# SinOncology/BreakID

Measured on AMD Instinct MI355X. Metric: M reads/s clustered+split-scanned, higher is better.
Workload: dtype int32/u8 (+f64 sd replay)

## Files before the change

breakid_amd/capi.py:

```python
from __future__ import annotations

import ctypes as C
import math
import os
import subprocess

import numpy as np

from . import abi

_HERE = os.path.dirname(os.path.abspath(__file__))
LIB_PATH = os.path.join(_HERE, "libbreakid_hip.so")
_LIB = None


class BreakIDError(RuntimeError):
    def __init__(self, code, msg):
        super().__init__("libbreakid_hip error %d: %s" % (code, msg))
        self.code = code


def build(verbose=False):
    cmd = ["make", "-C", os.path.join(_HERE, "csrc"), "-j8"]
    r = subprocess.run(cmd, capture_output=not verbose, text=True)
    if r.returncode != 0:
        raise RuntimeError("building libbreakid_hip.so failed:\n" + (r.stdout or "")[-4000:] + (r.stderr or "")[-4000:])


EXPORTS = ["bk_init", "bk_prepare_process", "bk_free", "bk_last_error", "bk_set_stream", "bk_sync", "bk_get_stream", "bk_upload_records", "bk_records", "bk_exclude_regions", "bk_isize_stats",
           "bk_discordant_pairs", "bk_mask_and_cluster", "bk_split_evidence", "bk_cluster_summary",
           "bk_split_breakpoints", "bk_normal_support", "bk_ref_support", "bk_genotype_call", "bk_clip_support", "bk_clip_reads", "bk_base_depth", "bk_clip_rescue", "bk_junctions", "bk_junction_sides", "bk_vcf_breakend_alt", "bk_evidence", "bk_unique_support", "bk_clip_consensus", "bk_junction_fit", "bk_locus_similarity", "bk_site_complexity", "bk_window_coverage", "bk_window_context", "bk_call_windows", "bk_fusion_frame", "bk_link_calls", "bk_locus_partners", "bk_call_partner_sites", "bk_fragment_sizes", "bk_fragment_bounds", "bk_known_calls", "bk_split_junctions", "bk_split_junction_counts", "bk_debug_split_junctions", "bk_cigar_gaps", "bk_cigar_gap_counts", "bk_clip_loci", "bk_clip_locus_counts", "bk_run", "bk_fetch", "bk_timing", "bk_timing_enable", "bk_timing_touched", "bk_group_stats", "bk_qname_hash", "bk_qname_check",
           "bk_bam_open", "bk_bam_header", "bk_bam_decode", "bk_bam_close", "bk_bam_extract", "bk_bam_names_free", "bk_bam_reads", "bk_reads_free", "bk_bam_decode_device", "bk_bam_decode_device_part", "bk_bam_decode_device_ctx", "bk_bam_dev_free", "bk_feed_release_caches", "bk_debug_bgzf_inflate", "bk_debug_std_sort", "bk_debug_scan", "bk_debug_radix_sort", "bk_debug_prims_info", "bk_sort_forms", "bk_debug_sort_info", "bk_debug_ahc", "bk_debug_points", "bk_debug_points_groups", "bk_debug_cluster_info", "bk_debug_stream_info", "bk_debug_stream_blocks", "bk_debug_cigar", "bk_debug_vote", "bk_debug_region", "bk_shard_begin", "bk_shard_get_stats", "bk_shard_set_stats",
           "bk_shard_sd_local", "bk_shard_sd_finish", "bk_shard_buffer", "bk_shard_set_buffer", "bk_shard_group_sizes",
           "bk_shard_own_groups", "bk_shard_route_candidates", "bk_shard_group_keys", "bk_shard_route_pairs", "bk_shard_group_pairs", "bk_shard_bp_cov", "bk_shard_bp_vote", "bk_shard_bp_vote_slice", "bk_shard_bp_set_voted", "bk_shard_bp_depth", "bk_shard_bp_finish"]


def lib():
    global _LIB
    if _LIB is None:
        if not os.path.exists(LIB_PATH):
            raise BreakIDError(abi.BK_ERR_NO_DEVICE, "libbreakid_hip.so is not built (run __graft_entry__.build()); "
                                                     "there is no CPU fallback")
        try:
            import torch
        except Exception:
            pass
        L = C.CDLL(LIB_PATH)
# ... 46 lines not shown
        L.bk_cigar_gaps.argtypes = [vp, C.c_int, C.c_uint32, C.c_uint32, C.c_uint32, C.c_uint32, C.POINTER(vp), u64p]
        L.bk_cigar_gap_counts.argtypes = [vp, u64p]
        L.bk_clip_loci.argtypes = [vp, vp, C.c_int, C.c_int, C.c_uint32, C.c_uint32, C.c_uint32, C.POINTER(vp), u64p]
        L.bk_clip_locus_counts.argtypes = [vp, u64p]
        L.bk_fetch.argtypes = [vp, C.c_int, C.POINTER(vp), u64p, C.POINTER(C.POINTER(C.c_uint64)), C.POINTER(C.c_uint32)]
        L.bk_timing.argtypes = [vp, C.POINTER(C.POINTER(C.c_char_p)), C.POINTER(C.POINTER(C.c_float)),
                                C.POINTER(C.POINTER(C.c_uint64)), C.POINTER(C.c_int)]
        L.bk_timing_enable.argtypes = [vp, C.c_int]
        L.bk_timing_touched.argtypes = [vp, C.POINTER(C.POINTER(C.c_uint64)), C.POINTER(C.c_int)]
        L.bk_debug_std_sort.argtypes = [vp, vp, vp, C.c_uint32, vp]
        L.bk_debug_scan.argtypes = [vp, C.c_int, vp, C.c_uint64, C.c_int, vp]
        L.bk_debug_radix_sort.argtypes = [vp, vp, vp, C.c_uint64, C.c_int, C.c_int, vp, vp]
        L.bk_debug_prims_info.argtypes = [u64p]
        L.bk_sort_forms.argtypes = [vp, u64p]
        L.bk_debug_sort_info.argtypes = [vp, u64p]
        L.bk_debug_ahc.argtypes = [vp, vp, vp, C.c_uint32, C.c_double, vp, vp, C.POINTER(C.c_uint32)]
        L.bk_debug_points.argtypes = [vp, C.c_int, vp, vp, C.c_uint32, C.c_double, vp, vp, C.POINTER(C.c_uint32)]
        L.bk_debug_points_groups.argtypes = [vp, C.c_int, vp, vp, vp, C.c_uint32, C.c_double, vp, vp, vp, C.POINTER(C.c_uint32)]
        L.bk_debug_cluster_info.argtypes = [u64p]
        L.bk_debug_stream_info.argtypes = [u64p]
        L.bk_debug_stream_blocks.argtypes = [C.c_uint]
        L.bk_debug_cigar.argtypes = [vp, C.c_uint32, vp, vp, vp, vp, vp, vp, vp]
        L.bk_debug_vote.argtypes = [vp, vp, C.c_uint32, vp, C.c_uint32, C.c_int32, C.c_int32, vp]
        L.bk_debug_region.argtypes = [vp, C.c_int32, C.c_uint32, C.c_uint32, C.c_uint64, vp, C.c_uint32, C.POINTER(C.c_uint32), C.POINTER(C.c_uint32),
                                      C.POINTER(C.c_uint32)]
        L.bk_shard_begin.argtypes = [vp, C.c_uint64, C.c_int]
        L.bk_shard_get_stats.argtypes = [vp, C.POINTER(abi.ShardStats)]
        L.bk_shard_set_stats.argtypes = [vp, C.POINTER(abi.ShardStats)]
        L.bk_shard_sd_local.argtypes = [vp, u64p, C.POINTER(vp), u64p]
        L.bk_shard_sd_finish.argtypes = [vp, vp, C.c_uint64, C.c_uint64, dp, dp]
# ... 108 lines not shown

def stream_info():
    out = (C.c_uint64 * 4)()
    rc = lib().bk_debug_stream_info(out)
    if rc != 0:
        raise BreakIDError(rc, "bk_debug_stream_info")
    return dict(zip(("STREAM_V", "ST_CAND_CAP", "ST_SA_CAP", "RESIDENT"), (int(v) for v in out)))


def stream_blocks(blocks):
    rc = lib().bk_debug_stream_blocks(int(blocks))
    if rc != 0:
        raise BreakIDError(rc, "bk_debug_stream_blocks")


def w_from(mean, sd):
    times = 2
    return times * math.sqrt(times) * (mean + 3 * sd)


def genotype_call(alt, ref):
    gt, gq, vaf = C.c_uint8(), C.c_uint8(), C.c_float()
    rc = lib().bk_genotype_call(int(alt), int(ref), C.byref(gt), C.byref(gq), C.byref(vaf))
    if rc != 0:
        raise BreakIDError(rc, "bk_genotype_call")
    return gt.value, gq.value, np.float32(vaf.value)


def junction_sides(row):
    a = np.zeros(1, abi.JUNCTION)
# ... 832 lines not shown
```

breakid_amd/csrc/api.hip:

```cpp
#include <algorithm>
#include <cmath>
#include <limits>
#include <cstring>
#include <numeric>

#include "bk_common.h"
#include "prims.h"
#include "stream.h"
#include "join.h"
#include "cluster.h"
#include "bp.h"
#include "normal.h"
#include "genotype.h"
#include "clip.h"
#include "junction.h"
#include "evidence.h"
#include "unique.h"
#include "consensus.h"
#include "jfit.h"
#include "locsim.h"
#include "seqcx.h"
#include "coverage.h"
#include "context.h"
#include "frame.h"
#include "link.h"
#include "partners.h"
#include "fragsize.h"
#include "known.h"
#include "sjcall.h"
#include "gaps.h"
#include "cliploci.h"
#include "exclude.h"
#include "ahc.h"
#include "lanes.h"
#include "bgzf_gpu.h"

namespace
{
thread_local std::string g_init_error;

uint64_t fnv64(const std::string &s)
{
  uint64_t h = 0xCBF29CE484222325ull;
  for (unsigned char c : s)
  {
    h ^= c;
    h *= 0x100000001B3ull;
  }
  return h;
// ... 27 lines not shown
  std::vector<int32_t> hdr_id_host;
  DevBuf d_tprefix, d_nhash, d_nid, d_own, d_hdr;
  NameTableDev names{};

  bk_soa rec{};
  DevBuf col[13];
  DevBuf d_side;
  DevBuf xcol[13];
  bool have_records = false;
  bool streamed = false;

  DevBuf d_counters, d_sd, d_cand, d_split_raw, d_split, d_sa_list;
  StreamCounters hc{};
  SdState hsd{};
  bool stream_done = false, splits_sorted = false;
  int mapq_min = 20;
  int stream_mapq = -1;
  uint64_t cand_cap = 0, split_cap = 0, sa_cap = 0;
  uint64_t rec_base = 0;
  std::vector<uint64_t> route_counts;
  JoinBufs jb2;
  const Cand *ext_cand = nullptr;
  const bk_split *ext_split = nullptr;
  bk_cluster *ext_clusters = nullptr;
  std::vector<uint8_t> own_groups;
  const Cand *cand_ptr() const { return ext_cand ? ext_cand : d_cand.get<Cand>(); }
  const bk_split *split_raw_ptr() const { return ext_split ? ext_split : d_split_raw.get<bk_split>(); }
  bk_cluster *clusters_ptr() const { return ext_clusters ? ext_clusters : d_clusters.get<bk_cluster>(); }
  SdBufs sdb;
  double mean = 0, sd = 0;
// ... 71 lines not shown
  ClipLociStats cll_stats;
  std::vector<struct bk_clip_locus> f_cll;

  prims::RadixBufs dbg_radix;
  DevBuf dbg_in, dbg_out, dbg_vals;

  std::vector<bk_pair> f_pairs[3];
  std::vector<uint64_t> f_off[3];
  std::vector<bk_split> f_splits;
  std::vector<bk_cluster> f_clusters;
  std::vector<int32_t> f_gkeys;
  std::vector<bk_group_stat> f_gstats;

  bool timing = false;
  std::vector<StageTimer> timers;
  Timing tout;

  void tick(const char *name, uint64_t bytes, bool begin, uint64_t touched = 0)
  {
    if (!timing) return;
    if (begin)
    {
      StageTimer t;
      t.name = name;
      t.bytes = bytes;
      t.touched = touched;
      HIP_CHECK(hipEventCreate(&t.a));
      HIP_CHECK(hipEventCreate(&t.b));
      HIP_CHECK(hipEventRecord(t.a, st));
      timers.push_back(t);
    }
    else
      HIP_CHECK(hipEventRecord(timers.back().b, st));
  }
};

static RecView rec_view(const bk_ctx *ctx)
{
  RecView r;
  r.n = ctx->rec.n;
  r.tid = ctx->rec.tid; r.pos = ctx->rec.pos; r.flag = ctx->rec.flag; r.mapq = ctx->rec.mapq;
  r.cigar_off = ctx->rec.cigar_off; r.cigar = ctx->rec.cigar;
  r.isize = ctx->rec.isize; r.aux_off = ctx->rec.aux_off;
  return r;
}

namespace
{
struct Scope
{
  bk_ctx *c;
  Scope(bk_ctx *c, const char *name, uint64_t bytes = 0, uint64_t touched = 0) : c(c) { c->tick(name, bytes, true, touched); }
  ~Scope()
  {
    try
    {
      c->tick("", 0, false);
    }
    catch (...)
    {
    }
  }
};

template <class F> int guarded(bk_ctx *ctx, F &&f)
{
  if (!ctx) return BK_ERR_ARG;
  try
  {
    HIP_CHECK(hipSetDevice(ctx->device));
    f();
    return BK_OK;
// ... 106 lines not shown
  (void) c->d_sa_list.as<uint32_t>(c->sa_cap);
}
bool stream_finish(bk_ctx *c)
{
  HIP_CHECK(hipMemcpyAsync(&c->hc, c->d_counters.get<StreamCounters>(), sizeof(StreamCounters), hipMemcpyDeviceToHost, c->st));
  HIP_CHECK(hipMemcpyAsync(&c->hsd, c->d_sd.get<SdState>(), sizeof(SdState), hipMemcpyDeviceToHost, c->st));
  HIP_CHECK(hipStreamSynchronize(c->st));
  if (c->hc.n_cand > c->cand_cap || c->hc.n_sa > c->sa_cap)
  {
    c->cand_cap = std::max<uint64_t>(c->cand_cap, c->hc.n_cand + 1024);
    c->sa_cap = std::max<uint64_t>(c->sa_cap, c->hc.n_sa + 1024);
    return false;
  }
  return true;
}
void stream_rare_path(bk_ctx *c)
{
  const uint64_t n = c->rec.n;
  if (c->timing && !c->timers.empty())
  {
    c->timers.back().bytes += 32ull * c->hc.n_cand + 4ull * c->hc.n_sa;
    c->timers.back().touched = 23ull * n + 4ull * c->rec.n_cigar_words + (c->rec.qcheck ? 60ull : 56ull) * c->hc.n_cand + 4ull * c->hc.n_sa;
  }
  if (c->hc.unsorted) throw bk_error(BK_ERR_UNSORTED, "records are not coordinate sorted (the reference requires an indexed, sorted BAM)");
  if (c->hc.n_sa > c->split_cap)
  {
    c->split_cap = c->hc.n_sa + 1024;
    (void) c->d_split_raw.as<bk_split>(c->split_cap);
  }
  StreamArgs a = stream_args(c, n);
  {
    Scope s(c, "k_split_records", c->rec.n_aux_bytes + 4ull * c->hc.n_sa);
    launch_split_records(a, c->hc.n_sa, c->st);
  }
  HIP_CHECK(hipMemcpyAsync(&c->hc, c->d_counters.get<StreamCounters>(), sizeof(StreamCounters), hipMemcpyDeviceToHost, c->st));
  HIP_CHECK(hipStreamSynchronize(c->st));
  if (c->timing && !c->timers.empty())
  {
    c->timers.back().bytes += 48ull * c->hc.n_split;
    c->timers.back().touched = c->timers.back().bytes + 40ull * c->hc.n_sa + 32ull * c->hc.n_split;
  }
  c->stream_done = true;
  c->stream_mapq = c->mapq_min;
  c->splits_sorted = false;
  c->stats_done = false;
}

void run_stream(bk_ctx *c)
{
  if (!c->have_records) throw bk_error(BK_ERR_ARG, "no records uploaded");
  const uint64_t n = c->rec.n;
  for (int attempt = 0; attempt < 3; ++attempt)
  {
    stream_prepare(c, n);
    {
      Scope s(c, "k_stream", 39ull * n + 4ull * c->rec.n_cigar_words);
      launch_stream(stream_args(c, n), c->st);
    }
    if (stream_finish(c)) break;
    if (c->timing && !c->timers.empty()) c->timers.pop_back();
    if (attempt == 2) throw bk_error(BK_ERR_LIMIT, "stream pass: output capacity");
  }
  stream_rare_path(c);
}

void ensure_splits_sorted(bk_ctx *c)
{
  if (c->splits_sorted) return;
  Scope s(c, "split_sort");
  bk_split *sorted = c->d_split.as<bk_split>(c->hc.n_split + 1);
  int bits = 0;
  if (!c->ext_split && c->rec_base == 0)
  {
    bits = 1;
    while (bits < 32 && (1ull << bits) < c->rec.n) ++bits;
  }
  sort_splits(const_cast<bk_split *>(c->split_raw_ptr()), c->hc.n_split, sorted, c->bb, c->st, bits);
  c->splits_sorted = true;
}
}

extern "C" {

void bk_prepare_process()
{
  static std::once_flag once;
  std::call_once(once, [] {
    const char *q = getenv("GPU_MAX_HW_QUEUES");
    stage_set_hw_queues(q ? atoi(q) : 4);
  });
}

// ... 310 lines not shown
        ctx->jb.rec_bits = bits;
      }
      join_candidates(ctx->cand_ptr(), ctx->hc.n_cand, w, ctx->d_tprefix.get<uint32_t>(), ctx->nt, ctx->jb, ctx->st, ctx->jr);
    }
    finish_groups(ctx, nullptr);
    ctx->clustered = false;
    ctx->joined = true;
    ctx->bp_done = false;
    ctx->sj_claims_valid = false;
    ctx->join_w = w;
    if (n_pairs) *n_pairs = ctx->jr.n_pairs;
    if (n_groups) *n_groups = ctx->jr.n_groups;
  });
}

int bk_mask_and_cluster(bk_ctx *ctx, double w, int fast, uint64_t *n_clustered)
{
  return guarded(ctx, [&] {
    const StageInput in{ctx->device, ctx->st, ctx->jr, ctx->gstart_host, ctx->own_groups,
                        [&](const char *name, const std::function<void()> &body) { Scope s(ctx, name); body(); }};
    ctx->summary_map = false;
    ctx->stage.run(in, w, fast);
    ctx->clustered = true;
    if (n_clustered) *n_clustered = ctx->stage.list.n;
  });
}

int bk_split_evidence(bk_ctx *ctx, uint64_t *n_tuples)
{
  return guarded(ctx, [&] {
    if (!ctx->stream_done) run_stream(ctx);
    ensure_splits_sorted(ctx);
    if (n_tuples) *n_tuples = ctx->hc.n_split;
  });
}

int bk_cluster_summary(bk_ctx *ctx, double w, uint64_t *n_clusters)
{
  return guarded(ctx, [&] {
    if (!ctx->clustered) throw bk_error(BK_ERR_ARG, "bk_cluster_summary: call bk_mask_and_cluster first");
    ctx->bp_done = false;
// ... 1271 lines not shown
{
  if (!mate_chr || !buf) return BK_ERR_ARG;
  const char br = mate_right ? '[' : ']';
  const std::string mate = br + std::string(mate_chr) + ":" + std::to_string(mate_pos) + br;
  const std::string alt = own_right ? mate + ref_base : ref_base + mate;
  if (alt.size() + 1 > cap) return BK_ERR_ARG;
  std::memcpy(buf, alt.c_str(), alt.size() + 1);
  return BK_OK;
}

int bk_run(bk_ctx *ctx, int mapq_min, int fast, double *w_out, uint64_t *n_valid)
{
  if (!ctx) return BK_ERR_ARG;
  if (ctx->stream_done && mapq_min != ctx->stream_mapq) ctx->stream_done = false;
  ctx->mapq_min = mapq_min;
  double mean, sd;
  int rc = bk_isize_stats(ctx, &mean, &sd);
  if (rc) return rc;
  const int times = 2;
  const double w = times * std::sqrt(times) * (mean + 3 * sd);
  if (w_out) *w_out = w;
  if ((rc = bk_discordant_pairs(ctx, mapq_min, w, nullptr, nullptr))) return rc;
  if ((rc = bk_mask_and_cluster(ctx, w, fast, nullptr))) return rc;
  if ((rc = bk_split_evidence(ctx, nullptr))) return rc;
  if ((rc = bk_cluster_summary(ctx, w, nullptr))) return rc;
  if ((rc = bk_split_breakpoints(ctx, w, n_valid))) return rc;
  return BK_OK;
}

int bk_fetch(bk_ctx *ctx, int stage, const void **data, uint64_t *count, const uint64_t **group_off, uint32_t *n_groups)
{
  return guarded(ctx, [&] {
    if (!data || !count) throw bk_error(BK_ERR_ARG, "bk_fetch: null output");
    const uint32_t ng = ctx->jr.n_groups;
    if (group_off) *group_off = nullptr;
    if (n_groups) *n_groups = 0;
    auto fetch_list = [&](int slot, const uint32_t *d_idx, const uint64_t *d_goff, const uint32_t *d_cl, uint64_t n) {
      std::vector<bk_pair> all(ctx->jr.n_pairs);
// ... 406 lines not shown
    if (!out) throw bk_error(BK_ERR_ARG, "bk_sort_forms: null output");
    ctx->stage.sort_forms(out);
  });
}

int bk_debug_sort_info(bk_ctx *ctx, uint64_t out[13])
{
  return guarded(ctx, [&] {
    if (!out) throw bk_error(BK_ERR_ARG, "bk_debug_sort_info: null output");
    static_assert(SORT_INFO_WORDS == 11, "bk_debug_sort_info: eleven words of the build, two of the last sort");
    std_sort_info(out);
    const SortEmuBufs &se = ctx->stage.cb().se;
    out[11] = se.last_heap[0];
    out[12] = se.last_heap[1];
  });
}

int bk_debug_ahc(bk_ctx *ctx, const uint32_t *x, const uint32_t *y, uint32_t n, double w, uint32_t *idx_out, int32_t *cluster_out, uint32_t *n_out)
{
  return guarded(ctx, [&] {
    if (!x || !y || !idx_out || !cluster_out || !n_out) throw bk_error(BK_ERR_ARG, "bk_debug_ahc: null argument");
    std::vector<bk_pair> hp(n);
    for (uint32_t i = 0; i < n; ++i)
    {
      memset(&hp[i], 0, sizeof(bk_pair));
      hp[i].x = x[i];
      hp[i].y = y[i];
    }
    DevBuf dp, dcl;
    PairList L;
// ... 435 lines not shown
```

breakid_amd/csrc/lanes.h:

```cpp
#pragma once
#include <functional>
#include <memory>

#include "join.h"
#include "cluster.h"
#include "ahc.h"

void stage_set_hw_queues(int n);

struct StageInput
{
  int device;
  hipStream_t st;
  const JoinResult &jr;
  const std::vector<uint64_t> &gstart_host;
  const std::vector<uint8_t> &own_groups;
  std::function<void(const char *name, const std::function<void()> &body)> timed;
};

struct ClusterStage
{
  SortService svc;
  std::vector<hipEvent_t> svc_probe;
  int svc_late = 0;
  bool svc_refused = false;
  struct Lane
  {
    ClusterBufs cb;
    PairList list, iso;
    DevBuf d_cluster;
    hipStream_t st = nullptr;
    ~Lane()
// ... 19 lines not shown
```

breakid_amd/csrc/lanes.hip:

```cpp
#include <algorithm>
#include <atomic>
#include <chrono>
#include <cmath>
#include <cstdio>
#include <numeric>
#include <thread>
#include <dirent.h>

#include "lanes.h"

static int g_hw_queues_at_init = 0;
void stage_set_hw_queues(int n) { g_hw_queues_at_init = n; }

static bool sort_service_on()
{
  static const bool on = !(getenv("BREAKID_SORT_SERVICE") && atoi(getenv("BREAKID_SORT_SERVICE")) == 0);
  return on;
}
constexpr int LANE_STREAMS_MAX = 4;
constexpr int SVC_STAGE_QUEUES = LANE_STREAMS_MAX + 3;
static bool lane_service(int fast) { return sort_service_on() && fast && g_hw_queues_at_init >= SVC_STAGE_QUEUES; }
static int stage_queues() { return std::max(1, g_hw_queues_at_init - 1); }
static int lanes_wanted(bool svc)
{
// ... 213 lines not shown
{
  uint32_t *ii = idx.as<uint32_t>(L.n + 1), *ig = gof ? gof->as<uint32_t>(L.n + 1) : nullptr;
  uint64_t *io = goff.as<uint64_t>((uint64_t) L.ng + 1);
  if (L.n) HIP_CHECK(hipMemcpyAsync(ii, L.idx.get<uint32_t>(), L.n * 4, hipMemcpyDeviceToDevice, st));
  if (L.n && ig) HIP_CHECK(hipMemcpyAsync(ig, L.gof.get<uint32_t>(), L.n * 4, hipMemcpyDeviceToDevice, st));
  if (L.ng) HIP_CHECK(hipMemcpyAsync(io, L.goff.get<uint64_t>(), ((uint64_t) L.ng + 1) * 8, hipMemcpyDeviceToDevice, st));
}
static void cluster_list(const bk_pair *pairs, PairList &L, double w, int fast, DevBuf &cl, ClusterBufs &cb, AhcBufs &ab, hipStream_t st)
{
  if (fast)
    fast_cluster_all(pairs, L, w, cl, cb, st);
  else
    ahc_cluster_all(pairs, L, w, cl, ab, cb, st);
}

using LanePlan = std::vector<int>;
static LanePlan plan_owned(const StageInput &in)
{
  const uint32_t ng = in.jr.n_groups;
  const bool owned_only = !in.own_groups.empty();
  if (owned_only && in.own_groups.size() != ng) throw bk_error(BK_ERR_ARG, "bk_shard_own_groups: group count changed");
  LanePlan p(ng, 0);
  for (uint32_t g = 0; owned_only && g < ng; ++g)
    if (!in.own_groups[g]) p[g] = -1;
  return p;
}
static LanePlan plan_blind(const StageInput &in, int K)
{
  const uint32_t ng = in.jr.n_groups;
  std::vector<uint32_t> order(ng);
  std::iota(order.begin(), order.end(), 0u);
  auto size_of = [&](uint32_t g) { return in.gstart_host[g + 1] - in.gstart_host[g]; };
  std::stable_sort(order.begin(), order.end(), [&](uint32_t a, uint32_t b) { return size_of(a) > size_of(b); });
  constexpr double wexp = 2.0;
  LanePlan p = plan_owned(in);
  std::vector<double> load(K, 0.0);
  for (uint32_t i = 0; i < ng; ++i)
  {
    const uint32_t g = order[i];
    if (p[g] < 0) continue;
    int l = 0;
    for (int k = 1; k < K; ++k)
      if (load[k] < load[l]) l = k;
    load[l] += std::pow((double) size_of(g), wexp);
    p[g] = l;
  }
  return p;
}
static LanePlan plan_observed(const std::vector<uint64_t> &sizes, const std::vector<uint32_t> &hx, const std::vector<uint32_t> &hy, int K)
{
  const uint32_t ng = (uint32_t) sizes.size();
  constexpr double per_pair = 0.001;
  auto heap_cost = [](uint32_t m) { return (double) m + (m > 40947u ? 1.0 * (double) (m - 40947u) : 0.0); };
  std::vector<uint32_t> order(ng);
  std::iota(order.begin(), order.end(), 0u);
  auto chain = [&](uint32_t g) { return heap_cost(hx[g]) + heap_cost(hy[g]); };
  std::stable_sort(order.begin(), order.end(), [&](uint32_t a, uint32_t b) {
    const double ca = chain(a), cb = chain(b);
    return ca != cb ? ca > cb : sizes[a] > sizes[b];
  });
  LanePlan p(ng, 0);
  std::vector<double> mx(K, 0.0), my(K, 0.0), pairs(K, 0.0);
  auto cost = [&](int l) { return mx[l] + my[l] + per_pair * pairs[l]; };
  for (uint32_t g : order)
  {
    int best = 0;
    double best_cost = 0;
    for (int l = 0; l < K; ++l)
    {
      const double c = std::max(mx[l], heap_cost(hx[g])) + std::max(my[l], heap_cost(hy[g])) + per_pair * (pairs[l] + (double) sizes[g]);
      if (l == 0 || c < best_cost || (c == best_cost && cost(l) < cost(best)))
      {
        best = l;
        best_cost = c;
      }
    }
    mx[best] = std::max(mx[best], heap_cost(hx[g]));
    my[best] = std::max(my[best], heap_cost(hy[g]));
    pairs[best] += (double) sizes[g];
    p[g] = best;
  }
  if (bk_debug("lanes"))
    for (int l = 0; l < K; ++l)
    {
      fprintf(stderr, "[lanes] lane %d: max heap x %.0f y %.0f, %.0f pairs, cost %.0f; heavy groups:", l, mx[l], my[l], pairs[l], cost(l));
      for (uint32_t g = 0; g < ng; ++g)
        if (p[g] == l && (hx[g] || hy[g])) fprintf(stderr, " %u(%u,%u)", g, hx[g], hy[g]);
      fprintf(stderr, "\n");
    }
  return p;
}
static uint32_t *upload_drop(const LanePlan &p, int K, DevBuf &buf, hipStream_t st)
{
  const size_t row = p.size() + 1;
  std::vector<uint32_t> drop((size_t) K * row, 0u);
  for (int l = 0; l < K; ++l)
    for (size_t g = 0; g + 1 < row; ++g) drop[(size_t) l * row + g] = p[g] == l ? 0u : 1u;
  uint32_t *d = buf.as<uint32_t>(drop.size() + 1);
  HIP_CHECK(hipMemcpyAsync(d, drop.data(), drop.size() * 4, hipMemcpyHostToDevice, st));
  HIP_CHECK(hipStreamSynchronize(st));
  return d;
}

static void group_lanes(ClusterStage &cs, const StageInput &in, double w, int fast)
// ... 97 lines not shown
    if (observe) cb.heavy_x.assign(ng, 0u);
    remove_isolated_end(pairs, lane(l).list, cb, lane_st(l));
    if (observe) cb.observe = false;
  };
  auto cluster_lane = [&](int l) {
    PairList &L = lane(l).list, &iso = lane(l).iso;
    iso.n = L.n;
    iso.ng = L.ng;
    snapshot_list(L, iso.idx, &iso.gof, iso.goff, lane_st(l));
    cluster_list(pairs, L, w, fast, lane(l).d_cluster, lane(l).cb, cs.ab, lane_st(l));
  };
  const auto tp0 = std::chrono::steady_clock::now();
  auto phase = [&](const char *what) {
    if (dbg) fprintf(stderr, "[lanes] %s at %.2f ms\n", what, std::chrono::duration<double, std::milli>(std::chrono::steady_clock::now() - tp0).count());
  };
  upload_plan(plan_blind(in, K));
  phase("plan uploaded");
  if (use_svc)
    in_lanes([&](int l) {
      mask_lane(l, false);
      cluster_lane(l);
    });
  else
  {
    in_lanes([&](int l) { mask_lane(l, true); });
    PairList &mid = cs.lane_mid;
    merge_all(&ClusterStage::Lane::list, mid, nullptr);
    std::vector<uint64_t> goff_h((size_t) ng + 1);
    HIP_CHECK(hipMemcpyAsync(goff_h.data(), mid.goff.get<uint64_t>(), ((size_t) ng + 1) * 8, hipMemcpyDeviceToHost, in.st));
    HIP_CHECK(hipStreamSynchronize(in.st));
    std::vector<uint64_t> sizes(ng);
    std::vector<uint32_t> hx(ng, 0u), hy(ng, 0u);
    for (uint32_t g = 0; g < ng; ++g) sizes[g] = goff_h[g + 1] - goff_h[g];
    for (int l = 0; l < K; ++l)
      for (uint32_t g = 0; g < ng; ++g)
      {
        hx[g] = std::max(hx[g], lane(l).cb.heavy_x[g]);
        hy[g] = std::max(hy[g], lane(l).cb.heavy_y[g]);
      }
    upload_plan(plan_observed(sizes, hx, hy, K));
    in_lanes([&](int l) {
      list_subset_ranges(mid, goff_h.data(), keep[l].data(), lane(l).list, lane_st(l));
      cluster_lane(l);
    });
  }
  phase("lanes done");
  svc_stage.finish();
  phase("service stopped");
  if (use_svc && bk_debug("lanes")) fprintf(stderr, "[svc] tasks: %u wide, %u narrow\n", cs.svc.stats[0], cs.svc.stats[1]);
  PairList &iso_m = cs.lane_iso_m;
  merge_all(&ClusterStage::Lane::iso, iso_m, nullptr);
  merge_all(&ClusterStage::Lane::list, cs.list, &cs.d_cluster);
  HIP_CHECK(hipStreamSynchronize(in.st));
  phase("lists merged");
  cs.iso_n = iso_m.n;
// ... 40 lines not shown
```

include/breakid_hip.h:

```cpp
#ifndef BREAKID_HIP_H
#define BREAKID_HIP_H

#include <stdint.h>
#include <stddef.h>

#ifdef __cplusplus
extern "C" {
#endif

#define BK_OK 0
#define BK_ERR_ARG (-1)
#define BK_ERR_HIP (-2)
#define BK_ERR_NO_DEVICE (-3)
#define BK_ERR_UNSORTED (-4)
#define BK_ERR_CIGAR (-5)
#define BK_ERR_IO (-6)
#define BK_ERR_LIMIT (-7)
#define BK_ERR_COLLISION (-8)

#define BK_MEM_HOST 0
#define BK_MEM_DEVICE 1

typedef struct bk_ctx bk_ctx;

// ... 350 lines not shown
int bk_shard_bp_vote_slice(bk_ctx *ctx, double w, const void *cov_total_dev, uint64_t lo, uint64_t hi, void **clusters_dev, void **voted_dev);
int bk_shard_bp_set_voted(bk_ctx *ctx, const void *voted_all_dev);
int bk_shard_bp_depth(bk_ctx *ctx, void **depth_dev, uint64_t *n);
int bk_shard_bp_finish(bk_ctx *ctx, const void *depth_total_dev);

int bk_debug_std_sort(bk_ctx *ctx, const uint32_t *key, const uint64_t *group_off, uint32_t n_groups, uint32_t *perm_out);

int bk_debug_scan(bk_ctx *ctx, int elem_bytes, const void *in, uint64_t n, int in_place, void *out);
int bk_debug_radix_sort(bk_ctx *ctx, const uint64_t *keys, const uint32_t *vals, uint64_t n, int begin_bit, int end_bit, uint64_t *keys_out, uint32_t *vals_out);
int bk_debug_prims_info(uint64_t out[4]);

int bk_sort_forms(bk_ctx *ctx, uint64_t out[3]);

int bk_debug_sort_info(bk_ctx *ctx, uint64_t out[13]);

int bk_debug_ahc(bk_ctx *ctx, const uint32_t *x, const uint32_t *y, uint32_t n, double w, uint32_t *idx_out, int32_t *cluster_out, uint32_t *n_out);

int bk_debug_points(bk_ctx *ctx, int mode, const uint32_t *x, const uint32_t *y, uint32_t n, double w, uint32_t *idx_out, int32_t *cluster_out, uint32_t *n_out);
int bk_debug_points_groups(bk_ctx *ctx, int mode, const uint32_t *x, const uint32_t *y, const uint64_t *group_off, uint32_t n_groups, double w, uint32_t *idx_out,
                           int32_t *cluster_out, uint64_t *goff_out, uint32_t *n_out);
int bk_debug_cluster_info(uint64_t out[2]);
int bk_debug_stream_info(uint64_t out[4]);
int bk_debug_stream_blocks(unsigned blocks);
int bk_debug_cigar(bk_ctx *ctx, uint32_t n, const uint8_t *kind, const uint32_t *c1_off, const uint8_t *c1, const uint32_t *c2_off, const uint8_t *c2, const int32_t *e,
                   int32_t *out6);
int bk_debug_vote(bk_ctx *ctx, const bk_split *side1, uint32_t n1, const bk_split *side2, uint32_t n2, int32_t p1_tid, int32_t p2_tid, int32_t *out3);
int bk_debug_region(bk_ctx *ctx, int32_t tid, uint32_t start, uint32_t end, uint64_t depth_pos, bk_split *out, uint32_t cap, uint32_t *n_out, uint32_t *cov_out,
                    uint32_t *depth_out);

typedef struct bk_bam bk_bam;
// ... 30 lines not shown
```

Baseline: 11730.

## Overlap split-record extraction with clustering lanes and model-based lane dealing

```diff
diff --git a/breakid_amd/capi.py b/breakid_amd/capi.py
--- a/breakid_amd/capi.py
+++ b/breakid_amd/capi.py
@@ -30,7 +30,7 @@
 EXPORTS = ["bk_init", "bk_prepare_process", "bk_free", "bk_last_error", "bk_set_stream", "bk_sync", "bk_get_stream", "bk_upload_records", "bk_records", "bk_exclude_regions", "bk_isize_stats",
            "bk_discordant_pairs", "bk_mask_and_cluster", "bk_split_evidence", "bk_cluster_summary",
            "bk_split_breakpoints", "bk_normal_support", "bk_ref_support", "bk_genotype_call", "bk_clip_support", "bk_clip_reads", "bk_base_depth", "bk_clip_rescue", "bk_junctions", "bk_junction_sides", "bk_vcf_breakend_alt", "bk_evidence", "bk_unique_support", "bk_clip_consensus", "bk_junction_fit", "bk_locus_similarity", "bk_site_complexity", "bk_window_coverage", "bk_window_context", "bk_call_windows", "bk_fusion_frame", "bk_link_calls", "bk_locus_partners", "bk_call_partner_sites", "bk_fragment_sizes", "bk_fragment_bounds", "bk_known_calls", "bk_split_junctions", "bk_split_junction_counts", "bk_debug_split_junctions", "bk_cigar_gaps", "bk_cigar_gap_counts", "bk_clip_loci", "bk_clip_locus_counts", "bk_run", "bk_fetch", "bk_timing", "bk_timing_enable", "bk_timing_touched", "bk_group_stats", "bk_qname_hash", "bk_qname_check",
-           "bk_bam_open", "bk_bam_header", "bk_bam_decode", "bk_bam_close", "bk_bam_extract", "bk_bam_names_free", "bk_bam_reads", "bk_reads_free", "bk_bam_decode_device", "bk_bam_decode_device_part", "bk_bam_decode_device_ctx", "bk_bam_dev_free", "bk_feed_release_caches", "bk_debug_bgzf_inflate", "bk_debug_std_sort", "bk_debug_scan", "bk_debug_radix_sort", "bk_debug_prims_info", "bk_sort_forms", "bk_debug_sort_info", "bk_debug_ahc", "bk_debug_points", "bk_debug_points_groups", "bk_debug_cluster_info", "bk_debug_stream_info", "bk_debug_stream_blocks", "bk_debug_cigar", "bk_debug_vote", "bk_debug_region", "bk_shard_begin", "bk_shard_get_stats", "bk_shard_set_stats",
+           "bk_bam_open", "bk_bam_header", "bk_bam_decode", "bk_bam_close", "bk_bam_extract", "bk_bam_names_free", "bk_bam_reads", "bk_reads_free", "bk_bam_decode_device", "bk_bam_decode_device_part", "bk_bam_decode_device_ctx", "bk_bam_dev_free", "bk_feed_release_caches", "bk_debug_bgzf_inflate", "bk_debug_std_sort", "bk_debug_scan", "bk_debug_radix_sort", "bk_debug_prims_info", "bk_sort_forms", "bk_debug_sort_info", "bk_debug_lane_plan", "bk_debug_ahc", "bk_debug_points", "bk_debug_points_groups", "bk_debug_cluster_info", "bk_debug_stream_info", "bk_debug_stream_blocks", "bk_debug_cigar", "bk_debug_vote", "bk_debug_region", "bk_shard_begin", "bk_shard_get_stats", "bk_shard_set_stats",
            "bk_shard_sd_local", "bk_shard_sd_finish", "bk_shard_buffer", "bk_shard_set_buffer", "bk_shard_group_sizes",
            "bk_shard_own_groups", "bk_shard_route_candidates", "bk_shard_group_keys", "bk_shard_route_pairs", "bk_shard_group_pairs", "bk_shard_bp_cov", "bk_shard_bp_vote", "bk_shard_bp_vote_slice", "bk_shard_bp_set_voted", "bk_shard_bp_depth", "bk_shard_bp_finish"]
 
@@ -107,6 +107,7 @@
         L.bk_debug_prims_info.argtypes = [u64p]
         L.bk_sort_forms.argtypes = [vp, u64p]
         L.bk_debug_sort_info.argtypes = [vp, u64p]
+        L.bk_debug_lane_plan.argtypes = [vp, vp, vp, C.c_uint32, C.c_int, C.c_int, vp, vp]
         L.bk_debug_ahc.argtypes = [vp, vp, vp, C.c_uint32, C.c_double, vp, vp, C.POINTER(C.c_uint32)]
         L.bk_debug_points.argtypes = [vp, C.c_int, vp, vp, C.c_uint32, C.c_double, vp, vp, C.POINTER(C.c_uint32)]
         L.bk_debug_points_groups.argtypes = [vp, C.c_int, vp, vp, vp, C.c_uint32, C.c_double, vp, vp, vp, C.POINTER(C.c_uint32)]
@@ -245,6 +246,23 @@
         raise BreakIDError(rc, "bk_debug_stream_blocks")
 
 
+LANE_PLAN_GREEDY, LANE_PLAN_MODEL, LANE_PLAN_EVAL = 0, 1, 2
+
+
+def lane_plan(pairs, hx, hy, K, which=LANE_PLAN_MODEL, plan=None):
+    pairs = np.ascontiguousarray(pairs, np.uint64)
+    hx = np.ascontiguousarray(hx, np.uint32)
+    hy = np.ascontiguousarray(hy, np.uint32)
+    assert len(pairs) == len(hx) == len(hy)
+    lane = np.zeros(len(pairs), np.int32) if plan is None else np.array(plan, np.int32)
+    assert len(lane) == len(pairs) and (which == LANE_PLAN_EVAL) == (plan is not None)
+    t = np.zeros(K, np.float64)
+    rc = lib().bk_debug_lane_plan(pairs.ctypes.data, hx.ctypes.data, hy.ctypes.data, len(pairs), int(K), int(which), lane.ctypes.data, t.ctypes.data)
+    if rc != 0:
+        raise BreakIDError(rc, "bk_debug_lane_plan")
+    return lane, t
+
+
 def w_from(mean, sd):
     times = 2
     return times * math.sqrt(times) * (mean + 3 * sd)
diff --git a/breakid_amd/csrc/api.hip b/breakid_amd/csrc/api.hip
--- a/breakid_amd/csrc/api.hip
+++ b/breakid_amd/csrc/api.hip
@@ -33,6 +33,7 @@
 #include "exclude.h"
 #include "ahc.h"
 #include "lanes.h"
+#include "lane_plan.h"
 #include "bgzf_gpu.h"
 
 namespace
@@ -90,6 +91,7 @@
   StreamCounters hc{};
   SdState hsd{};
   bool stream_done = false, splits_sorted = false;
+  bool defer_split = false, split_pending = false;
   int mapq_min = 20;
   int stream_mapq = -1;
   uint64_t cand_cap = 0, split_cap = 0, sa_cap = 0;
@@ -191,11 +193,14 @@
 
   bool timing = false;
   std::vector<StageTimer> timers;
+  std::vector<StageTimer> side_timers;
   Timing tout;
 
-  void tick(const char *name, uint64_t bytes, bool begin, uint64_t touched = 0)
+  void tick(const char *name, uint64_t bytes, bool begin, uint64_t touched = 0, hipStream_t on = nullptr, std::vector<StageTimer> *into = nullptr)
   {
     if (!timing) return;
+    if (!on) on = st;
+    if (!into) into = &timers;
     if (begin)
     {
       StageTimer t;
@@ -204,11 +209,11 @@
       t.touched = touched;
       HIP_CHECK(hipEventCreate(&t.a));
       HIP_CHECK(hipEventCreate(&t.b));
-      HIP_CHECK(hipEventRecord(t.a, st));
-      timers.push_back(t);
+      HIP_CHECK(hipEventRecord(t.a, on));
+      into->push_back(t);
     }
     else
-      HIP_CHECK(hipEventRecord(timers.back().b, st));
+      HIP_CHECK(hipEventRecord(into->back().b, on));
   }
 };
 
@@ -227,12 +232,17 @@
 struct Scope
 {
   bk_ctx *c;
-  Scope(bk_ctx *c, const char *name, uint64_t bytes = 0, uint64_t touched = 0) : c(c) { c->tick(name, bytes, true, touched); }
+  hipStream_t on;
+  std::vector<StageTimer> *into;
+  Scope(bk_ctx *c, const char *name, uint64_t bytes = 0, uint64_t touched = 0, hipStream_t on = nullptr, std::vector<StageTimer> *into = nullptr) : c(c), on(on), into(into)
+  {
+    c->tick(name, bytes, true, touched, on, into);
+  }
   ~Scope()
   {
     try
     {
-      c->tick("", 0, false);
+      c->tick("", 0, false, 0, on, into);
     }
     catch (...)
     {
@@ -369,6 +379,24 @@
   }
   return true;
 }
+void split_records(bk_ctx *c, hipStream_t st, std::vector<StageTimer> *side)
+{
+  StreamArgs a = stream_args(c, c->rec.n);
+  {
+    Scope s(c, "k_split_records", c->rec.n_aux_bytes + 4ull * c->hc.n_sa, 0, st, side);
+    launch_split_records(a, c->hc.n_sa, st);
+  }
+  HIP_CHECK(hipMemcpyAsync(&c->hc, c->d_counters.get<StreamCounters>(), sizeof(StreamCounters), hipMemcpyDeviceToHost, st));
+  HIP_CHECK(hipStreamSynchronize(st));
+  std::vector<StageTimer> &ts = side ? *side : c->timers;
+  if (c->timing && !ts.empty())
+  {
+    ts.back().bytes += 48ull * c->hc.n_split;
+    ts.back().touched = ts.back().bytes + 40ull * c->hc.n_sa + 32ull * c->hc.n_split;
+  }
+  c->split_pending = false;
+}
+
 void stream_rare_path(bk_ctx *c)
 {
   const uint64_t n = c->rec.n;
@@ -383,18 +411,8 @@
     c->split_cap = c->hc.n_sa + 1024;
     (void) c->d_split_raw.as<bk_split>(c->split_cap);
   }
-  StreamArgs a = stream_args(c, n);
-  {
-    Scope s(c, "k_split_records", c->rec.n_aux_bytes + 4ull * c->hc.n_sa);
-    launch_split_records(a, c->hc.n_sa, c->st);
-  }
-  HIP_CHECK(hipMemcpyAsync(&c->hc, c->d_counters.get<StreamCounters>(), sizeof(StreamCounters), hipMemcpyDeviceToHost, c->st));
-  HIP_CHECK(hipStreamSynchronize(c->st));
-  if (c->timing && !c->timers.empty())
-  {
-    c->timers.back().bytes += 48ull * c->hc.n_split;
-    c->timers.back().touched = c->timers.back().bytes + 40ull * c->hc.n_sa + 32ull * c->hc.n_split;
-  }
+  c->split_pending = c->defer_split;
+  if (!c->split_pending) split_records(c, c->st, nullptr);
   c->stream_done = true;
   c->stream_mapq = c->mapq_min;
   c->splits_sorted = false;
@@ -419,10 +437,12 @@
   stream_rare_path(c);
 }
 
-void ensure_splits_sorted(bk_ctx *c)
-{
+void ensure_splits_sorted(bk_ctx *c, hipStream_t st = nullptr, std::vector<StageTimer> *side = nullptr)
+{
+  if (!st) st = c->st;
+  if (c->split_pending) split_records(c, st, side);
   if (c->splits_sorted) return;
-  Scope s(c, "split_sort");
+  Scope s(c, "split_sort", 0, 0, st, side);
   bk_split *sorted = c->d_split.as<bk_split>(c->hc.n_split + 1);
   int bits = 0;
   if (!c->ext_split && c->rec_base == 0)
@@ -430,7 +450,7 @@
     bits = 1;
     while (bits < 32 && (1ull << bits) < c->rec.n) ++bits;
   }
-  sort_splits(const_cast<bk_split *>(c->split_raw_ptr()), c->hc.n_split, sorted, c->bb, c->st, bits);
+  sort_splits(const_cast<bk_split *>(c->split_raw_ptr()), c->hc.n_split, sorted, c->bb, st, bits);
   c->splits_sorted = true;
 }
 }
@@ -771,17 +791,28 @@
   });
 }
 
-int bk_mask_and_cluster(bk_ctx *ctx, double w, int fast, uint64_t *n_clustered)
+static int mask_and_cluster(bk_ctx *ctx, double w, int fast, uint64_t *n_clustered, const std::function<void(hipStream_t)> &idle_work)
 {
   return guarded(ctx, [&] {
     const StageInput in{ctx->device, ctx->st, ctx->jr, ctx->gstart_host, ctx->own_groups,
-                        [&](const char *name, const std::function<void()> &body) { Scope s(ctx, name); body(); }};
+                        [&](const char *name, const std::function<void()> &body) { Scope s(ctx, name); body(); }, idle_work};
     ctx->summary_map = false;
+    struct SideTimers
+    {
+      bk_ctx *c;
+      ~SideTimers()
+      {
+        c->timers.insert(c->timers.end(), c->side_timers.begin(), c->side_timers.end());
+        c->side_timers.clear();
+      }
+    } side{ctx};
     ctx->stage.run(in, w, fast);
     ctx->clustered = true;
     if (n_clustered) *n_clustered = ctx->stage.list.n;
   });
 }
+
+int bk_mask_and_cluster(bk_ctx *ctx, double w, int fast, uint64_t *n_clustered) { return mask_and_cluster(ctx, w, fast, n_clustered, nullptr); }
 
 int bk_split_evidence(bk_ctx *ctx, uint64_t *n_tuples)
 {
@@ -2083,14 +2114,27 @@
   if (!ctx) return BK_ERR_ARG;
   if (ctx->stream_done && mapq_min != ctx->stream_mapq) ctx->stream_done = false;
   ctx->mapq_min = mapq_min;
+  struct Deferred
+  {
+    bk_ctx *c;
+    ~Deferred()
+    {
+      c->defer_split = false;
+      if (c->split_pending) c->stream_done = c->split_pending = false;
+    }
+  } deferred{ctx};
+  ctx->defer_split = fast != 0;
   double mean, sd;
   int rc = bk_isize_stats(ctx, &mean, &sd);
+  ctx->defer_split = false;
   if (rc) return rc;
   const int times = 2;
   const double w = times * std::sqrt(times) * (mean + 3 * sd);
   if (w_out) *w_out = w;
   if ((rc = bk_discordant_pairs(ctx, mapq_min, w, nullptr, nullptr))) return rc;
-  if ((rc = bk_mask_and_cluster(ctx, w, fast, nullptr))) return rc;
+  std::function<void(hipStream_t)> idle_work;
+  if (fast) idle_work = [ctx](hipStream_t st) { ensure_splits_sorted(ctx, st, &ctx->side_timers); };
+  if ((rc = mask_and_cluster(ctx, w, fast, nullptr, idle_work))) return rc;
   if ((rc = bk_split_evidence(ctx, nullptr))) return rc;
   if ((rc = bk_cluster_summary(ctx, w, nullptr))) return rc;
   if ((rc = bk_split_breakpoints(ctx, w, n_valid))) return rc;
@@ -2527,6 +2571,33 @@
     out[11] = se.last_heap[0];
     out[12] = se.last_heap[1];
   });
+}
+
+int bk_debug_lane_plan(const uint64_t *pairs, const uint32_t *hx, const uint32_t *hy, uint32_t ng, int K, int which, int *lane_out, double *lane_T_out)
+{
+  if (K < 1 || K > 26 || which < 0 || which > 2 || !lane_out || (ng && (!pairs || !hx || !hy))) return BK_ERR_ARG;
+  const std::vector<uint64_t> sizes(pairs, pairs + ng);
+  const std::vector<uint32_t> vx(hx, hx + ng), vy(hy, hy + ng);
+  const LaneModel model;
+  std::vector<double> T(K, 0.0);
+  LanePlan p;
+  if (which == 2)
+  {
+    p.assign(lane_out, lane_out + ng);
+    for (int l : p)
+      if (l < 0 || l >= K) return BK_ERR_ARG;
+    lane_plan_eval(model, p, sizes, vx, vy, K, T.data());
+  }
+  else if (which == 1)
+    p = plan_observed_model(model, sizes, vx, vy, K, T.data());
+  else
+  {
+    p = plan_observed_greedy(sizes, vx, vy, K);
+    lane_plan_eval(model, p, sizes, vx, vy, K, T.data());
+  }
+  std::copy(p.begin(), p.end(), lane_out);
+  if (lane_T_out) std::copy(T.begin(), T.end(), lane_T_out);
+  return BK_OK;
 }
 
 int bk_debug_ahc(bk_ctx *ctx, const uint32_t *x, const uint32_t *y, uint32_t n, double w, uint32_t *idx_out, int32_t *cluster_out, uint32_t *n_out)
diff --git a/breakid_amd/csrc/lane_plan.h b/breakid_amd/csrc/lane_plan.h
--- /dev/null
+++ b/breakid_amd/csrc/lane_plan.h
@@ -0,0 +1,232 @@
+#pragma once
+#include <algorithm>
+#include <cmath>
+#include <cstdint>
+#include <numeric>
+#include <vector>
+
+using LanePlan = std::vector<int>;
+
+static inline LanePlan plan_blind(const std::vector<uint64_t> &gstart, LanePlan p, int K)
+{
+  const uint32_t ng = (uint32_t) p.size();
+  std::vector<uint32_t> order(ng);
+  std::iota(order.begin(), order.end(), 0u);
+  auto size_of = [&](uint32_t g) { return gstart[g + 1] - gstart[g]; };
+  std::stable_sort(order.begin(), order.end(), [&](uint32_t a, uint32_t b) { return size_of(a) > size_of(b); });
+  constexpr double wexp = 2.0;
+  std::vector<double> load(K, 0.0);
+  for (uint32_t i = 0; i < ng; ++i)
+  {
+    const uint32_t g = order[i];
+    if (p[g] < 0) continue;
+    int l = 0;
+    for (int k = 1; k < K; ++k)
+      if (load[k] < load[l]) l = k;
+    load[l] += std::pow((double) size_of(g), wexp);
+    p[g] = l;
+  }
+  return p;
+}
+
+static inline LanePlan plan_observed_greedy(const std::vector<uint64_t> &sizes, const std::vector<uint32_t> &hx, const std::vector<uint32_t> &hy, int K)
+{
+  const uint32_t ng = (uint32_t) sizes.size();
+  constexpr double per_pair = 0.001;
+  auto heap_cost = [](uint32_t m) { return (double) m + (m > 40947u ? 1.0 * (double) (m - 40947u) : 0.0); };
+  std::vector<uint32_t> order(ng);
+  std::iota(order.begin(), order.end(), 0u);
+  auto chain = [&](uint32_t g) { return heap_cost(hx[g]) + heap_cost(hy[g]); };
+  std::stable_sort(order.begin(), order.end(), [&](uint32_t a, uint32_t b) {
+    const double ca = chain(a), cb = chain(b);
+    return ca != cb ? ca > cb : sizes[a] > sizes[b];
+  });
+  LanePlan p(ng, 0);
+  std::vector<double> mx(K, 0.0), my(K, 0.0), pairs(K, 0.0);
+  auto cost = [&](int l) { return mx[l] + my[l] + per_pair * pairs[l]; };
+  for (uint32_t g : order)
+  {
+    int best = 0;
+    double best_cost = 0;
+    for (int l = 0; l < K; ++l)
+    {
+      const double c = std::max(mx[l], heap_cost(hx[g])) + std::max(my[l], heap_cost(hy[g])) + per_pair * (pairs[l] + (double) sizes[g]);
+      if (l == 0 || c < best_cost || (c == best_cost && cost(l) < cost(best)))
+      {
+        best = l;
+        best_cost = c;
+      }
+    }
+    mx[best] = std::max(mx[best], heap_cost(hx[g]));
+    my[best] = std::max(my[best], heap_cost(hy[g]));
+    pairs[best] += (double) sizes[g];
+    p[g] = best;
+  }
+  return p;
+}
+
+struct LaneModel
+{
+  double t_spine = 1.39;
+  double a = 0.169e-3;
+  double b = 0.50e-6;
+  double c0 = 1.59;
+  double c1 = 0.357e-6;
+  uint32_t cap32 = 40873;
+  double heap_cost(uint32_t m) const { return (double) m + (m > cap32 ? (double) (m - cap32) : 0.0); }
+  double sort(uint32_t H, double P) const { return std::max(t_spine + a * heap_cost(H), b * P); }
+  double lane(uint32_t Hx, uint32_t Hy, double P) const { return sort(Hy, P) + sort(Hx, P) + c0 + c1 * P; }
+};
+constexpr int LANE_HEAVY_TOP = 8;
+
+struct LaneLoad
+{
+  uint32_t hx = 0, hy = 0;
+  double pairs = 0;
+  void add(uint32_t x, uint32_t y, uint64_t n)
+  {
+    hx = std::max(hx, x);
+    hy = std::max(hy, y);
+    pairs += (double) n;
+  }
+};
+static inline double lane_plan_eval(const LaneModel &M, const LanePlan &p, const std::vector<uint64_t> &sizes, const std::vector<uint32_t> &hx, const std::vector<uint32_t> &hy, int K,
+                                    double *T)
+{
+  std::vector<LaneLoad> L(K);
+  for (size_t g = 0; g < p.size(); ++g)
+    if (p[g] >= 0 && p[g] < K) L[p[g]].add(hx[g], hy[g], sizes[g]);
+  double worst = 0;
+  for (int l = 0; l < K; ++l)
+  {
+    const double t = M.lane(L[l].hx, L[l].hy, L[l].pairs);
+    if (T) T[l] = t;
+    worst = std::max(worst, t);
+  }
+  return worst;
+}
+
+static inline LanePlan plan_observed_model(const LaneModel &M, const std::vector<uint64_t> &sizes, const std::vector<uint32_t> &hx, const std::vector<uint32_t> &hy, int K, double *T)
+{
+  const uint32_t ng = (uint32_t) sizes.size();
+  LanePlan p(ng, 0);
+  if (K > 1 && ng)
+  {
+    std::vector<uint32_t> heavy, light;
+    for (uint32_t g = 0; g < ng; ++g) (std::max(hx[g], hy[g]) > 0 ? heavy : light).push_back(g);
+    auto chain = [&](uint32_t g) { return M.heap_cost(hx[g]) + M.heap_cost(hy[g]); };
+    std::stable_sort(heavy.begin(), heavy.end(), [&](uint32_t a, uint32_t b) {
+      const double ca = chain(a), cb = chain(b);
+      return ca != cb ? ca > cb : sizes[a] > sizes[b];
+    });
+    std::stable_sort(light.begin(), light.end(), [&](uint32_t a, uint32_t b) { return sizes[a] > sizes[b]; });
+    std::vector<LaneLoad> L(K);
+    auto lane_T = [&](const LaneLoad &l) { return M.lane(l.hx, l.hy, l.pairs); };
+    double left = 0;
+    for (uint32_t g = 0; g < ng; ++g) left += (double) sizes[g];
+    auto bound = [&](double span, double sum) { return std::max(span, (sum + M.c1 * left) / K); };
+    const int top = (int) std::min<size_t>(heavy.size(), LANE_HEAVY_TOP);
+    for (int i = 0; i < top; ++i) left -= (double) sizes[heavy[i]];
+    {
+      int cur[LANE_HEAVY_TOP] = {0}, best[LANE_HEAVY_TOP] = {0};
+      double best_span = -1, best_sum = 0;
+      std::vector<LaneLoad> stack((size_t) (top + 1) * K);
+      auto at = [&](int d) { return stack.data() + (size_t) d * K; };
+      int d = 0, open[LANE_HEAVY_TOP + 1] = {0};
+      if (top) cur[0] = -1;
+      while (top && d >= 0)
+      {
+        if (++cur[d] > std::min(open[d], K - 1))
+        {
+          --d;
+          continue;
+        }
+        std::copy(at(d), at(d) + K, at(d + 1));
+        const uint32_t g = heavy[d];
+        at(d + 1)[cur[d]].add(hx[g], hy[g], sizes[g]);
+        open[d + 1] = std::max(open[d], cur[d] + 1);
+        if (d + 1 < top)
+        {
+          cur[++d] = -1;
+          continue;
+        }
+        double span = 0, sum = 0;
+        for (int l = 0; l < K; ++l)
+        {
+          const double t = lane_T(at(d + 1)[l]);
+          span = std::max(span, t);
+          sum += t;
+        }
+        span = bound(span, sum);
+        if (best_span < 0 || span < best_span || (span == best_span && sum < best_sum))
+        {
+          best_span = span;
+          best_sum = sum;
+          std::copy(cur, cur + top, best);
+        }
+      }
+      for (int i = 0; i < top; ++i)
+      {
+        p[heavy[i]] = best[i];
+        L[best[i]].add(hx[heavy[i]], hy[heavy[i]], sizes[heavy[i]]);
+      }
+    }
+    std::vector<double> t(K);
+    for (int l = 0; l < K; ++l) t[l] = lane_T(L[l]);
+    for (size_t i = (size_t) top; i < heavy.size(); ++i)
+    {
+      const uint32_t g = heavy[i];
+      left -= (double) sizes[g];
+      int pick = 0;
+      double pick_span = 0, pick_grow = 0, pick_t = 0;
+      for (int l = 0; l < K; ++l)
+      {
+        LaneLoad with = L[l];
+        with.add(hx[g], hy[g], sizes[g]);
+        const double tl = lane_T(with);
+        double span = tl, sum = tl;
+        for (int k = 0; k < K; ++k)
+          if (k != l)
+          {
+            span = std::max(span, t[k]);
+            sum += t[k];
+          }
+        span = bound(span, sum);
+        const double grow = tl - t[l];
+        if (l == 0 || span < pick_span || (span == pick_span && grow < pick_grow))
+        {
+          pick = l;
+          pick_span = span;
+          pick_grow = grow;
+          pick_t = tl;
+        }
+      }
+      L[pick].add(hx[g], hy[g], sizes[g]);
+      t[pick] = pick_t;
+      p[g] = pick;
+    }
+    for (uint32_t g : light)
+    {
+      int pick = 0;
+      double pick_t = 0;
+      for (int l = 0; l < K; ++l)
+      {
+        LaneLoad with = L[l];
+        with.add(0u, 0u, sizes[g]);
+        const double tl = lane_T(with);
+        if (l == 0 || tl < pick_t)
+        {
+          pick = l;
+          pick_t = tl;
+        }
+      }
+      L[pick].add(0u, 0u, sizes[g]);
+      t[pick] = pick_t;
+      p[g] = pick;
+    }
+    const LanePlan old = plan_observed_greedy(sizes, hx, hy, K);
+    if (lane_plan_eval(M, old, sizes, hx, hy, K, nullptr) < lane_plan_eval(M, p, sizes, hx, hy, K, nullptr)) p = old;
+  }
+  lane_plan_eval(M, p, sizes, hx, hy, K, T);
+  return p;
+}
diff --git a/breakid_amd/csrc/lanes.h b/breakid_amd/csrc/lanes.h
--- a/breakid_amd/csrc/lanes.h
+++ b/breakid_amd/csrc/lanes.h
@@ -16,6 +16,7 @@
   const std::vector<uint64_t> &gstart_host;
   const std::vector<uint8_t> &own_groups;
   std::function<void(const char *name, const std::function<void()> &body)> timed;
+  std::function<void(hipStream_t)> idle_work;
 };
 
 struct ClusterStage
diff --git a/breakid_amd/csrc/lanes.hip b/breakid_amd/csrc/lanes.hip
--- a/breakid_amd/csrc/lanes.hip
+++ b/breakid_amd/csrc/lanes.hip
@@ -3,11 +3,13 @@
 #include <chrono>
 #include <cmath>
 #include <cstdio>
+#include <cstring>
 #include <numeric>
 #include <thread>
 #include <dirent.h>
 
 #include "lanes.h"
+#include "lane_plan.h"
 
 static int g_hw_queues_at_init = 0;
 void stage_set_hw_queues(int n) { g_hw_queues_at_init = n; }
@@ -251,7 +253,6 @@
     ahc_cluster_all(pairs, L, w, cl, ab, cb, st);
 }
 
-using LanePlan = std::vector<int>;
 static LanePlan plan_owned(const StageInput &in)
 {
   const uint32_t ng = in.jr.n_groups;
@@ -260,71 +261,6 @@
   LanePlan p(ng, 0);
   for (uint32_t g = 0; owned_only && g < ng; ++g)
     if (!in.own_groups[g]) p[g] = -1;
-  return p;
-}
-static LanePlan plan_blind(const StageInput &in, int K)
-{
-  const uint32_t ng = in.jr.n_groups;
-  std::vector<uint32_t> order(ng);
-  std::iota(order.begin(), order.end(), 0u);
-  auto size_of = [&](uint32_t g) { return in.gstart_host[g + 1] - in.gstart_host[g]; };
-  std::stable_sort(order.begin(), order.end(), [&](uint32_t a, uint32_t b) { return size_of(a) > size_of(b); });
-  constexpr double wexp = 2.0;
-  LanePlan p = plan_owned(in);
-  std::vector<double> load(K, 0.0);
-  for (uint32_t i = 0; i < ng; ++i)
-  {
-    const uint32_t g = order[i];
-    if (p[g] < 0) continue;
-    int l = 0;
-    for (int k = 1; k < K; ++k)
-      if (load[k] < load[l]) l = k;
-    load[l] += std::pow((double) size_of(g), wexp);
-    p[g] = l;
-  }
-  return p;
-}
-static LanePlan plan_observed(const std::vector<uint64_t> &sizes, const std::vector<uint32_t> &hx, const std::vector<uint32_t> &hy, int K)
-{
-  const uint32_t ng = (uint32_t) sizes.size();
-  constexpr double per_pair = 0.001;
-  auto heap_cost = [](uint32_t m) { return (double) m + (m > 40947u ? 1.0 * (double) (m - 40947u) : 0.0); };
-  std::vector<uint32_t> order(ng);
-  std::iota(order.begin(), order.end(), 0u);
-  auto chain = [&](uint32_t g) { return heap_cost(hx[g]) + heap_cost(hy[g]); };
-  std::stable_sort(order.begin(), order.end(), [&](uint32_t a, uint32_t b) {
-    const double ca = chain(a), cb = chain(b);
-    return ca != cb ? ca > cb : sizes[a] > sizes[b];
-  });
-  LanePlan p(ng, 0);
-  std::vector<double> mx(K, 0.0), my(K, 0.0), pairs(K, 0.0);
-  auto cost = [&](int l) { return mx[l] + my[l] + per_pair * pairs[l]; };
-  for (uint32_t g : order)
-  {
-    int best = 0;
-    double best_cost = 0;
-    for (int l = 0; l < K; ++l)
-    {
-      const double c = std::max(mx[l], heap_cost(hx[g])) + std::max(my[l], heap_cost(hy[g])) + per_pair * (pairs[l] + (double) sizes[g]);
-      if (l == 0 || c < best_cost || (c == best_cost && cost(l) < cost(best)))
-      {
-        best = l;
-        best_cost = c;
-      }
-    }
-    mx[best] = std::max(mx[best], heap_cost(hx[g]));
-    my[best] = std::max(my[best], heap_cost(hy[g]));
-    pairs[best] += (double) sizes[g];
-    p[g] = best;
-  }
-  if (bk_debug("lanes"))
-    for (int l = 0; l < K; ++l)
-    {
-      fprintf(stderr, "[lanes] lane %d: max heap x %.0f y %.0f, %.0f pairs, cost %.0f; heavy groups:", l, mx[l], my[l], pairs[l], cost(l));
-      for (uint32_t g = 0; g < ng; ++g)
-        if (p[g] == l && (hx[g] || hy[g])) fprintf(stderr, " %u(%u,%u)", g, hx[g], hy[g]);
-      fprintf(stderr, "\n");
-    }
   return p;
 }
 static uint32_t *upload_drop(const LanePlan &p, int K, DevBuf &buf, hipStream_t st)
@@ -452,7 +388,7 @@
   auto phase = [&](const char *what) {
     if (dbg) fprintf(stderr, "[lanes] %s at %.2f ms\n", what, std::chrono::duration<double, std::milli>(std::chrono::steady_clock::now() - tp0).count());
   };
-  upload_plan(plan_blind(in, K));
+  upload_plan(plan_blind(in.gstart_host, plan_owned(in), K));
   phase("plan uploaded");
   if (use_svc)
     in_lanes([&](int l) {
@@ -461,7 +397,17 @@
     });
   else
   {
-    in_lanes([&](int l) { mask_lane(l, true); });
+    std::atomic<bool> idle_taken{false};
+    in_lanes([&](int l) {
+      mask_lane(l, true);
+      static const bool idle_off = getenv("BREAKID_LANE_IDLE") && atoi(getenv("BREAKID_LANE_IDLE")) == 0;
+      if (!in.idle_work || idle_off) return;
+      HIP_CHECK(hipStreamSynchronize(lane_st(l)));
+      if (idle_taken.exchange(true)) return;
+      const auto ti0 = std::chrono::steady_clock::now();
+      in.idle_work(lane_st(l));
+      if (dbg) fprintf(stderr, "[lanes] lane %d ran the idle work, queued in %.2f ms\n", l, std::chrono::duration<double, std::milli>(std::chrono::steady_clock::now() - ti0).count());
+    });
     PairList &mid = cs.lane_mid;
     merge_all(&ClusterStage::Lane::list, mid, nullptr);
     std::vector<uint64_t> goff_h((size_t) ng + 1);
@@ -476,7 +422,40 @@
         hx[g] = std::max(hx[g], lane(l).cb.heavy_x[g]);
         hy[g] = std::max(hy[g], lane(l).cb.heavy_y[g]);
       }
-    upload_plan(plan_observed(sizes, hx, hy, K));
+    static const bool greedy_deal = getenv("BREAKID_LANE_DEAL") && !strcmp(getenv("BREAKID_LANE_DEAL"), "greedy");
+    static const uint32_t cap32 = [] {
+      uint64_t info[SORT_INFO_WORDS];
+      std_sort_info(info);
+      return (uint32_t) info[10];
+    }();
+    LaneModel model;
+    model.cap32 = cap32;
+    std::vector<double> lane_T(K, 0.0);
+    const auto tplan0 = std::chrono::steady_clock::now();
+    LanePlan deal;
+    if (greedy_deal)
+    {
+      deal = plan_observed_greedy(sizes, hx, hy, K);
+      lane_plan_eval(model, deal, sizes, hx, hy, K, lane_T.data());
+    }
+    else
+      deal = plan_observed_model(model, sizes, hx, hy, K, lane_T.data());
+    const double plan_ms = std::chrono::duration<double, std::milli>(std::chrono::steady_clock::now() - tplan0).count();
+    if (bk_debug("lanes"))
+    {
+      fprintf(stderr, "[lanes] part-2 deal (%s) of %u groups planned in %.3f ms\n", greedy_deal ? "greedy" : "model", ng, plan_ms);
+      for (int l = 0; l < K; ++l)
+      {
+        LaneLoad ll;
+        for (uint32_t g = 0; g < ng; ++g)
+          if (deal[g] == l) ll.add(hx[g], hy[g], sizes[g]);
+        fprintf(stderr, "[lanes] lane %d: max heap x %u y %u, %.0f pairs, modelled T %.2f ms; heavy groups:", l, ll.hx, ll.hy, ll.pairs, lane_T[l]);
+        for (uint32_t g = 0; g < ng; ++g)
+          if (deal[g] == l && (hx[g] || hy[g])) fprintf(stderr, " %u(%u,%u)", g, hx[g], hy[g]);
+        fprintf(stderr, "\n");
+      }
+    }
+    upload_plan(deal);
     in_lanes([&](int l) {
       list_subset_ranges(mid, goff_h.data(), keep[l].data(), lane(l).list, lane_st(l));
       cluster_lane(l);
diff --git a/include/breakid_hip.h b/include/breakid_hip.h
--- a/include/breakid_hip.h
+++ b/include/breakid_hip.h
@@ -388,6 +388,8 @@
 
 int bk_debug_sort_info(bk_ctx *ctx, uint64_t out[13]);
 
+int bk_debug_lane_plan(const uint64_t *pairs, const uint32_t *hx, const uint32_t *hy, uint32_t ng, int K, int which, int *lane_out, double *lane_T_out);
+
 int bk_debug_ahc(bk_ctx *ctx, const uint32_t *x, const uint32_t *y, uint32_t n, double w, uint32_t *idx_out, int32_t *cluster_out, uint32_t *n_out);
 
 int bk_debug_points(bk_ctx *ctx, int mode, const uint32_t *x, const uint32_t *y, uint32_t n, double w, uint32_t *idx_out, int32_t *cluster_out, uint32_t *n_out);
```

New measurement: 12220, median of 6. 1.04x the previous value.
